# Matrixeigs/PowerSystemsReliabilityAssessment

Hardware: AMD Instinct MI355X
Metric: Monte Carlo DC-OPF scenarios/sec (RTS-24 HL2 non-sequential) (higher is better)
Workload: dtype f64

## Files before the change

powersystemsreliabilityassessment_amd/_lib.py:

```python
from __future__ import annotations

import ctypes as C
import os
import subprocess

from . import _abi

_CSRC = os.path.join(os.path.dirname(os.path.abspath(__file__)), "csrc")
LIB_PATH = os.environ.get("RELMC_LIB_PATH") or os.path.join(_CSRC, "librelmc.so")

EXPORTS = [
    "relmc_ctx_create", "relmc_ctx_destroy", "relmc_last_error", "relmc_version",
    "relmc_solver_opts_default", "relmc_nsq_opts_default", "relmc_case_load",
    "relmc_case_thresholds", "relmc_mc_sampling", "relmc_mc_sampling_dev",
    "relmc_mc_simulation", "relmc_mc_simulation_dev", "relmc_nsq_accumulate", "relmc_nsq_accumulate_distinct",
    "relmc_last_kernel_ms", "relmc_acc_zero", "relmc_acc_merge", "relmc_nsq_indices",
    "relmc_nsq_run", "relmc_hl1_load", "relmc_hl1_nsq", "relmc_hl1_seq_load", "relmc_hl1_seq", "relmc_hl1_seq_events", "relmc_hl1_seq_sweep",
    "relmc_hl1_plan_load", "relmc_hl1_plan", "relmc_hl1_area_load", "relmc_hl1_area", "relmc_hl1_area_tie_outages",
    "relmc_comm_unique_id", "relmc_comm_init", "relmc_comm_allreduce_acc", "relmc_comm_destroy", "relmc_comm_set_host_allreduce", "relmc_comm_info",
    "relmc_db_reset", "relmc_nsq_db_batch", "relmc_db_accumulate", "relmc_db_size", "relmc_db_export", "relmc_db_import",
    "relmc_seq_load", "relmc_seq_mcsampling", "relmc_seq_mcsimulation", "relmc_seq_years", "relmc_retry_stats", "relmc_retry_overflow", "relmc_retry_dense_stats", "relmc_case_order",
    "relmc_case_order_hint", "relmc_tune_order",
    "relmc_comm_set_timeout", "relmc_comm_allreduce_f64", "relmc_comm_set_host_allreduce_f64", "relmc_device_pci_bus_id", "relmc_seq_opts_default", "relmc_seq_run",
    "relmc_is_ratios", "relmc_is_sampling", "relmc_is_sampling_dev", "relmc_nsq_is_accumulate", "relmc_is_acc_zero", "relmc_is_acc_merge", "relmc_nsq_is_indices",
# ... 165 lines not shown
    L.relmc_is_acc_zero.argtypes = [C.POINTER(_abi.IsAcc)]
    L.relmc_is_acc_zero.restype = None
    L.relmc_is_acc_merge.argtypes = [C.POINTER(_abi.IsAcc), C.POINTER(_abi.IsAcc)]
    L.relmc_is_acc_merge.restype = None
    L.relmc_nsq_is_indices.argtypes = [C.POINTER(_abi.IsAcc), C.c_int32, C.c_int32, C.c_double, C.POINTER(_abi.IsIndices)]
    L.relmc_nsq_is_indices.restype = None
    L.relmc_is_tune_opts_default.argtypes = [C.POINTER(_abi.IsTuneOpts)]
    L.relmc_is_tune_opts_default.restype = None
    L.relmc_nsq_is_tune.argtypes = [vp, C.POINTER(_abi.IsTuneOpts), dp, C.POINTER(_abi.IsTuneReport)]
    L.relmc_nsq_is_tune.restype = C.c_int32
    L.relmc_is_run_opts_default.argtypes = [C.POINTER(_abi.IsRunOpts)]
    L.relmc_is_run_opts_default.restype = None
    L.relmc_nsq_is_run.argtypes = [vp, C.POINTER(_abi.IsRunOpts), C.POINTER(_abi.IsRunResult)]
    L.relmc_nsq_is_run.restype = C.c_int32
    if hasattr(L, "relmc_debug_mc_simulation_dense"):
        L.relmc_debug_mc_simulation_dense.argtypes = [vp, u8p, C.c_int64, C.c_void_p, dp, dp, i32p, i32p]
        L.relmc_debug_mc_simulation_dense.restype = C.c_int32
    L.relmc_case_order.argtypes = [vp, i32p, i32p]
    L.relmc_case_order.restype = C.c_int32
    L.relmc_case_order_hint.argtypes = [vp, i32p, C.c_int32]
    L.relmc_case_order_hint.restype = C.c_int32
    L.relmc_tune_order.argtypes = [C.c_void_p, C.c_int32, C.c_uint64, i32p, i32p, i32p]
    L.relmc_tune_order.restype = C.c_int32
    L.relmc_db_export.argtypes = [vp, C.c_int64, C.c_int64, u8p, _abi.c_int64_p, dp, i32p, dp, i32p, i32p, u8p]
    L.relmc_db_export.restype = C.c_int32
    L.relmc_db_import.argtypes = [vp, C.c_void_p, C.c_int64, u8p, _abi.c_int64_p, dp, dp, i32p, i32p, u8p]
    L.relmc_db_import.restype = C.c_int32
    if hasattr(L, "relmc_debug_screen_states"):
        L.relmc_debug_screen_states.argtypes = [vp, u8p, dp, C.c_int64, u8p]
        L.relmc_debug_screen_states.restype = C.c_int32
    if hasattr(L, "relmc_debug_stretch_len"):
        L.relmc_debug_stretch_len.argtypes = [C.c_int64, C.c_int64, C.c_double, C.c_double, C.c_int64, i32p]
        L.relmc_debug_stretch_len.restype = C.c_int64
    if hasattr(L, "relmc_debug_set"):
        L.relmc_debug_set.argtypes = [vp, C.c_char_p, C.c_int32]
        L.relmc_debug_set.restype = C.c_int32
    if hasattr(L, "relmc_debug_tail_plan"):
        L.relmc_debug_tail_plan.argtypes = [C.c_int64, C.c_int32, C.c_void_p, C.c_void_p, C.c_void_p, C.c_void_p]
        L.relmc_debug_tail_plan.restype = C.c_int32
        L.relmc_debug_tail_groups.argtypes = [vp, _abi.c_int64_p, i32p]
        L.relmc_debug_tail_groups.restype = C.c_int32
    if hasattr(L, "relmc_dpp_probe"):
        L.relmc_dpp_probe.argtypes = [vp, dp, dp]
        L.relmc_dpp_probe.restype = C.c_int32
    _lib = L
    return L
```

powersystemsreliabilityassessment_amd/csrc/relmc_ctx.h:

```cpp
#pragma once
#include <hip/hip_runtime.h>

#include <cmath>
#include <cstdint>
#include <functional>
#include <string>
#include <vector>

#include "../../include/relmc.h"
#include "relmc_dev.h"

struct relmc_switches {
    bool no_retry = false;
    bool retry_dense_first = false;
    bool nsq_no_stretch = false;
    bool db_no_probe = false;
    bool dynamic_shape = false;
    bool static_tail = false;
};

namespace relmc_host {
template <class T, bool Pinned = false>
class Buffer {
public:
// ... 151 lines not shown
        c->retry_units = units; c->retry_converged = converged; c->retry_dense_units = dense_units; c->retry_dense_converged = dense_converged; c->retry_overflow = overflow;
    }
};

namespace relmc_host {

using namespace relmc;

extern const char* const kNoCtx;
int fail(relmc_ctx* ctx, int code, const std::string& msg);
bool verbose();
inline int64_t first_non_finite(const double* x, int64_t n)
{
    for (int64_t i = 0; i < n; ++i)
        if (!std::isfinite(x[i])) return i;
    return -1;
}

#define HIP_TRY(ctx, expr)                                                                                   \
    do {                                                                                                     \
        hipError_t e_ = (expr);                                                                              \
        if (e_ != hipSuccess)                                                                                \
            return ::relmc_host::fail(ctx, RELMC_ERR_HIP, std::string(#expr) + ": " + hipGetErrorString(e_)); \
    } while (0)

struct SymOpts {
    const int32_t* order_hint = nullptr; int n_hint = 0;
    int place_moves = 100;
    long place_ww = 1;
    bool no_quarter = false, no_half = false, no_bwd_half = false, no_bus_map = false;
    int scen_pad4 = 0;
    int model_leaf_free = -1;
};
struct SymGeom { uint32_t stash_off = 0, scen_doubles = 0, lds_bytes = 0; long conflict_before = 0, conflict_after = 0; };
SymOpts sym_opts_default();
template <class TL>
int case_symbolic(const relmc_case_desc* d, DevCaseT<TL>& C, int order_variant, const SymOpts& so, SymGeom& geom, std::string& err);
extern template int case_symbolic<Tile24>(const relmc_case_desc*, DevCaseT<Tile24>&, int, const SymOpts&, SymGeom&, std::string&);
extern template int case_symbolic<Tile96>(const relmc_case_desc*, DevCaseT<Tile96>&, int, const SymOpts&, SymGeom&, std::string&);
inline bool fits_tile24(const relmc_case_desc* d)
{
    return d->nb <= Tile24::NBT && d->nl <= Tile24::NLT && d->ng + d->nd <= Tile24::NIT && d->ng + d->nl <= Tile24::NCOMPMAX;
}

EvalArgs make_args(const relmc_solver_opts& o);
int launch_eval(relmc_ctx* ctx, int mode, EvalArgs& a, int* rows_out, hipEvent_t ev_start = nullptr, hipEvent_t ev_stop = nullptr, int alt = 0);
int launch_finalize(relmc_ctx* ctx, int rows);
int finish_timing(relmc_ctx* ctx);
int case_load_image(relmc_ctx* ctx, const relmc_case_desc* d, int order_variant);
inline int mask_words(const relmc_ctx* ctx) { return ctx->tile == 0 ? Tile24::OW : Tile96::OW; }

#ifndef RELMC_TAIL_GROUPS
#define RELMC_TAIL_GROUPS 8
#endif
constexpr int kTailGroups = RELMC_TAIL_GROUPS;
struct TailPlan {
    int64_t ngroups, waves; int T;
    TailPlan(int64_t n, int64_t waves_) : ngroups((n + Tile24::SPW - 1) / Tile24::SPW), waves(waves_), T(waves_ > 0 && ngroups / waves_ >= 2 * kTailGroups ? kTailGroups : 0) {}
    int64_t begin(int64_t w) const { return ngroups * w / waves; }
    int64_t end(int64_t w) const { return ngroups * (w + 1) / waves; }
    int64_t cut(int64_t w) const { return end(w) - T; }
    int64_t items() const { return waves * T; }
    int64_t owner(int64_t p) const { return p % waves; }
    int64_t group(int64_t p) const { return end(p % waves) - T + p / waves; }
};

constexpr uint32_t kFailCapMin = 4096, kFailCapSteady = 1u << 20, kFailCapMax = 1u << 26;
// ... 58 lines not shown
```

powersystemsreliabilityassessment_amd/csrc/relmc_dev.h:

```cpp
#pragma once
#include <stdint.h>

namespace relmc {

template <int RW_, int BS_, int LS_, int IS_, int NCOMPMAX_, int MAXPASS_, int MAXOFF_, int WPB_>
struct TileT {
    static constexpr int RW = RW_;
    static constexpr int BS = BS_;
    static constexpr int LS = LS_;
    static constexpr int IS = IS_;
    static constexpr int NBT = BS_ * RW_;
    static constexpr int NLT = LS_ * RW_;
    static constexpr int NIT = IS_ * RW_;
    static constexpr int SPW = 64 / RW_;
    static constexpr int NCOMPMAX = NCOMPMAX_;
    static constexpr int OW = NCOMPMAX_ / 32;
    static constexpr int MAXPASS = MAXPASS_;
    static constexpr int MAXOFF = MAXOFF_;
    static constexpr int WPB = WPB_;
    static_assert(BS_ <= 2 && LS_ <= 3 && IS_ <= 4, "the per-lane flag word has room for 2 bus, 3 line and 4 injection slots");
};
using Tile24 = TileT<16, 2, 3, 4, 128, 96, 160, 4>;
using Tile96 = TileT<64, 2, 2, 3, 256, 64, 320, 8>;
constexpr int DEGMAX = 8;
constexpr int BINJMAX = 8;

constexpr uint32_t LF_EXISTS = 1u, LF_OWNER = 2u, LF_LIMITED = 4u;
constexpr uint32_t IK_NONE = 0u, IK_REAL = 1u, IK_VIRTUAL = 2u;

template <class TL>
struct DevCaseT {
    static constexpr int NBT = TL::NBT, NLT = TL::NLT, NIT = TL::NIT, NCOMPMAX = TL::NCOMPMAX, MAXPASS = TL::MAXPASS, MAXOFF = TL::MAXOFF, ROWL = TL::RW;
    int32_t nb, ng, nl, nd, ninj, ncomp, ref_bus, noff;
    double base_mva, total_load;
    uint32_t exist_mask;
    uint32_t nws;
    uint16_t off_rhs, off_p;
    uint16_t npass, npass_upd, npass_inv, nzero;
    uint16_t maxdeg, maxinj, base_connected, npass_updq;
    uint16_t maxdeg_s[2], maxinj_s[2];
    uint16_t npass_updh, pad3[3];
    uint64_t bwd_half;
    uint64_t b_line8[NBT];
    uint64_t b_inj8[NBT];
    double b_bsum[NBT];
    double l_b[NLT];
    double l_rate[NLT];
    uint32_t l_info[NLT];
    int32_t l_partner[NLT];
    uint16_t l_blk[NLT];
    alignas(16) double i_tab[NIT][4];
    uint32_t i_info[NIT];
    uint8_t b_nline[NBT];
    uint8_t b_line[NBT][DEGMAX];
    uint8_t b_ninj[NBT];
    uint8_t b_inj[NBT][BINJMAX];
    int16_t b_vinj[NBT];
    uint8_t b_ext[NBT];
    uint8_t b_lane[NBT];
    uint8_t b_int[NBT];
    uint32_t thr[NCOMPMAX];
// ... 153 lines not shown
```

powersystemsreliabilityassessment_amd/csrc/relmc_kernels.hip:

```cpp
#include "relmc_devfn.h"
#include "relmc_shape_rts24.h"

namespace relmc {


constexpr int kPrioBit = 12;
constexpr int kMinWaves = 2;
#define DINF __builtin_inf()
#define RELOAD_FENCE() __asm__ volatile("" ::: "memory")
#define SLOT_FENCE() __builtin_amdgcn_sched_barrier(0)
#ifdef RELMC_PASS_NOUNROLL
#define PASS_LOOP _Pragma("nounroll")
#else
#define PASS_LOOP
#endif
constexpr int kPfMask = 0xc0;
constexpr int kPfMaskWide = 0xc6;
#define PFSITE(k) (((PF_MASK >> (k)) & 1) != 0)
#ifdef RELMC_PHASE_TIMING
#define PT_DECL unsigned long long pt_[8] = {0, 0, 0, 0, 0, 0, 0, 0}; unsigned long long pt0_ = __builtin_readcyclecounter();
#define PT_MARK(k) { const unsigned long long n_ = __builtin_readcyclecounter(); pt_[k] += n_ - pt0_; pt0_ = n_; }
#define PT_FLUSH if (a.timing && lane == 0) { for (int k = 0; k < 8; ++k) a.timing[((size_t)blockIdx.x * WPB + (tid >> 6)) * 8 + k] = pt_[k]; }
#else
#define PT_DECL
#define PT_MARK(k)
#define PT_FLUSH
#endif
#if defined(RELMC_PHASE_TIMING) && defined(RELMC_PT_INIT)
#undef PT_MARK
#define PT_MARK(k) { const unsigned long long n_ = __builtin_readcyclecounter(); pt_[(k) == 7 ? 7 : 6] += n_ - pt0_; pt0_ = n_; }
#define PT_IMARK(k) { const unsigned long long n_ = __builtin_readcyclecounter(); pt_[k] += n_ - pt0_; pt0_ = n_; }
#else
#define PT_IMARK(k)
#endif

template <int MODE_, class TL, class SH = ShapeDynamic>
__global__ void __launch_bounds__(64 * TL::WPB, kMinWaves) relmc_eval_kernel(const DevCaseT<TL>* __restrict__ gcase, const EvalArgs a)
{
    constexpr int MODE = MODE_ == 5 ? 0 : (MODE_ == 6 ? 4 : MODE_);
    constexpr bool DENSE = MODE_ == 6;
    constexpr int PAIR_MASK = TL::RW == 16 ? kRpairMask : kRpairMaskWide;
#define PAIRSITE(k) (((PAIR_MASK >> (k)) & 1) != 0)
    constexpr int PF_MASK = TL::RW == 16 ? kPfMask : kPfMaskWide;
    constexpr int RW = TL::RW, BS = TL::BS, LS = TL::LS, IS = TL::IS, NBT = TL::NBT, WPB = TL::WPB, SPW = TL::SPW, OW = TL::OW;
    using DevCase = DevCaseT<TL>;
    using Partial = PartialT<TL>;
    extern __shared__ __attribute__((aligned(16))) unsigned char smem[];
    constexpr uint32_t OPT_BYTES = 128;
    double* const OPT = reinterpret_cast<double*>(smem);
#define A_(k, name) OPT[k]
    DevCase& C = *reinterpret_cast<DevCase*>(smem + OPT_BYTES);
    const DevCase& TASKSRC = *gcase;
    const DevCase& TABL = C;
    const DevCase& TABI = (RW == 64) ? *gcase : C;
    const DevCase& TABG = (RW == 64) ? *gcase : C;
    const int tid = threadIdx.x, lane = tid & 63, rlane = lane & (RW - 1), row = tid / RW;
    const uint32_t case_bytes = a.case_bytes;
    {
        const uint32_t* src = reinterpret_cast<const uint32_t*>(gcase);
        uint32_t* dst = reinterpret_cast<uint32_t*>(smem + OPT_BYTES);
        if (tid == 0) { OPT[0] = a.feastol; OPT[1] = a.gradtol; OPT[2] = a.comptol; OPT[3] = a.costtol; OPT[4] = a.xi; OPT[5] = a.sigma;
                        OPT[6] = a.z0; OPT[7] = a.alpha_min; OPT[8] = a.max_stepsize; OPT[9] = a.fail_threshold; }
        for (uint32_t i = tid; i < case_bytes / 4; i += 64 * WPB) dst[i] = src[i];
    }
    __syncthreads();
    double* const W = reinterpret_cast<double*>(smem + OPT_BYTES + ((case_bytes + 15u) & ~15u)) + (size_t)row * SHAPE(scen_doubles, a.scen_doubles);
    const int nlp = SHAPE(nl, C.nl), nip = SHAPE(ninj, C.ninj);
    double* const LR = W;
    double* const IR = W + 4 * (nlp + 1);
    const int maxdeg0 = SHAPE(maxdeg0, C.maxdeg_s[0]), maxdeg1 = SHAPE(maxdeg1, C.maxdeg_s[1]), maxinj0 = SHAPE(maxinj0, C.maxinj_s[0]), maxinj1 = SHAPE(maxinj1, C.maxinj_s[1]);
    double* const Stash = W + SHAPE(stash_off, a.stash_off) + 2 * rlane;
    const double* const StashJ = W + SHAPE(stash_off, a.stash_off);
    double* const Lam = W + SHAPE(stash_off, a.stash_off) + 2 * IS * RW + 2;
    uint32_t* const OB = reinterpret_cast<uint32_t*>(Lam + NBT);

    const int ng = SHAPE(ng, C.ng), ncomp = C.ncomp, nb = SHAPE(nb, C.nb);
// ... 741 lines not shown
                        for (int i = k + rlane; i < n; i += RW) { const double v = __builtin_fabs(A[(size_t)i * n1 + k]); if (v > best) { best = v; bi = i; } }
                        const double mx = row_max<RW>(best);
                        const uint32_t cand = (best == mx) ? (uint32_t)bi : (uint32_t)n;
                        const int p = (int)row_min_u32<RW>(cand);
                        if (!(mx > 0.0)) { singular_k = true; break; }
                        if (p != k) for (int j = k + rlane; j <= n; j += RW) { const double u = A[(size_t)k * n1 + j], v = A[(size_t)p * n1 + j]; A[(size_t)k * n1 + j] = v; A[(size_t)p * n1 + j] = u; }
                        __threadfence_block();
                        const double rp = 1.0 / A[(size_t)k * n1 + k];
                        for (int i = k + 1 + rlane; i < n; i += RW) Fm[i] = A[(size_t)i * n1 + k] * rp;
                        RELOAD_FENCE();
                        for (int i = k + 1; i < n; ++i) {
                            const double f = Fm[i];
                            if (f != 0.0) for (int j = k + 1 + rlane; j <= n; j += RW) A[(size_t)i * n1 + j] = A[(size_t)i * n1 + j] - f * A[(size_t)k * n1 + j];
                        }
                        __threadfence_block();
                    }
                    for (int k = n - 1; k >= 0 && !singular_k; --k) {
                        double sdot = 0.0;
                        for (int j = k + 1 + rlane; j < n; j += RW) sdot = __builtin_fma(A[(size_t)k * n1 + j], Fm[j], sdot);
                        sdot = row_sum<RW>(sdot);
                        if (rlane == 0) Fm[k] = (A[(size_t)k * n1 + n] - sdot) / A[(size_t)k * n1 + k];
                        RELOAD_FENCE();
                    }
                    double xs[(2 * NBT + RW - 1) / RW];
#pragma unroll
                    for (int q = 0; q < (2 * NBT + RW - 1) / RW; ++q) { const int e = rlane + RW * q; xs[q] = e < n ? (singular_k ? __builtin_nan("") : Fm[e]) : 0.0; }
                    RELOAD_FENCE();
#pragma unroll
                    for (int q = 0; q < (2 * NBT + RW - 1) / RW; ++q) { const int e = rlane + RW * q; if (e < n) W[off_rhs + e] = xs[q]; }
                    RELOAD_FENCE();
                } else {
                unsigned char* const W8 = reinterpret_cast<unsigned char*>(W);
#define WP(off) reinterpret_cast<double*>(W8 + (off))
                uint2 dsc = *reinterpret_cast<const uint2*>(&TASKSRC.task[0][rlane][0]);
                PASS_LOOP
                for (int p = 0; p < npuf; ++p) {
                    const uint2 nxt = *reinterpret_cast<const uint2*>(&TASKSRC.task[p + 1][rlane][0]);
                    if ((dsc.x & 0xffffu) != 0xffffu) {
                        const bool vec = (dsc.x & 0x8000u) != 0;
                        double* T = WP(dsc.x & 0x7fffu);
                        const double* Wa = WP(dsc.x >> 16);
                        const double* Wb = WP(dsc.y & 0xffffu);
                        const double* D = WP(dsc.y >> 16);
                        const d2 dA = ld2(D); const double dBy = D[3];
                        const d2 a0 = ld2(Wa), b0 = ld2(Wb), b1 = ld2(Wb + 2);
                        d2 t0 = ld2(T);
                        const double pm = dA.x, pb = dA.y, pe = -dBy;
                        const double q = frcp(__builtin_fma(pm, pe, pb * pb));
                        const double P00 = pe * q, P01 = pb * q, P11 = -pm * q;
                        const double g00 = __builtin_fma(a0.x, P00, a0.y * P01), g01 = __builtin_fma(a0.x, P01, a0.y * P11);
                        t0.x -= __builtin_fma(g00, b0.x, g01 * b0.y); t0.y -= __builtin_fma(g00, b1.x, g01 * b1.y);
                        st2(T, t0.x, t0.y);
                        if (!vec) {
                            const d2 a1 = ld2(Wa + 2);
                            d2 t1 = ld2(T + 2);
                            const double g10 = __builtin_fma(a1.x, P00, a1.y * P01), g11 = __builtin_fma(a1.x, P01, a1.y * P11);
                            t1.x -= __builtin_fma(g10, b0.x, g11 * b0.y); t1.y -= __builtin_fma(g10, b1.x, g11 * b1.y);
                            st2(T + 2, t1.x, t1.y);
                        }
                    }
                    dsc = nxt;
                }
                PASS_LOOP
                for (int p = npuf; p < npuh; ++p) {
                    const uint2 nxt = *reinterpret_cast<const uint2*>(&TASKSRC.task[p + 1][rlane][0]);
                    if ((dsc.x & 0xffffu) != 0xffffu) {
                        double* T = WP(dsc.x & 0xffffu);
                        const double* Wa = WP(dsc.x >> 16);
                        const double* Wb = WP(dsc.y & 0xffffu);
                        const double* D = WP(dsc.y >> 16);
                        const d2 dA = ld2(D); const double dBy = D[3];
                        const d2 a0 = ld2(Wa), b0 = ld2(Wb), b1 = ld2(Wb + 2);
                        d2 t0 = ld2(T);
                        const double pm = dA.x, pb = dA.y, pe = -dBy;
                        const double q = frcp(__builtin_fma(pm, pe, pb * pb));
                        const double P00 = pe * q, P01 = pb * q, P11 = -pm * q;
                        const double g00 = __builtin_fma(a0.x, P00, a0.y * P01), g01 = __builtin_fma(a0.x, P01, a0.y * P11);
                        t0.x -= __builtin_fma(g00, b0.x, g01 * b0.y); t0.y -= __builtin_fma(g00, b1.x, g01 * b1.y);
                        st2(T, t0.x, t0.y);
                    }
                    dsc = nxt;
                }
                PASS_LOOP
                for (int p = npuh; p < npu; ++p) {
                    const uint2 nxt = *reinterpret_cast<const uint2*>(&TASKSRC.task[p + 1][rlane][0]);
                    if ((dsc.x & 0xffffu) != 0xffffu) {
                        double* T = WP(dsc.x & 0xffffu);
                        const double* Wa = WP(dsc.x >> 16);
                        const double* Wb = WP(dsc.y & 0xffffu);
                        const double* D = WP(dsc.y >> 16);
                        const d2 dA = ld2(D); const double dBy = D[3];
                        const d2 a0 = ld2(Wa), b0 = ld2(Wb);
                        double t = *T;
                        const double pm = dA.x, pb = dA.y, pe = -dBy;
                        const double q = frcp(__builtin_fma(pm, pe, pb * pb));
                        const double P00 = pe * q, P01 = pb * q, P11 = -pm * q;
                        const double g0 = __builtin_fma(a0.x, P00, a0.y * P01), g1 = __builtin_fma(a0.x, P01, a0.y * P11);
                        t -= __builtin_fma(g0, b0.x, g1 * b0.y);
                        *T = t;
                    }
                    dsc = nxt;
                }
                PT_MARK(4)
                PASS_LOOP
                for (int p = npu; p < npu + npi; ++p) {
                    const uint2 nxt = *reinterpret_cast<const uint2*>(&TASKSRC.task[p + 1][rlane][0]);
                    if ((dsc.x & 0xffffu) != 0xffffu) {
                        double* D = WP(dsc.x & 0xffffu);
                        double* Y = WP(dsc.x >> 16);
                        const d2 dA = ld2(D), y = ld2(Y); const double dBy = D[3];
                        const double pm = dA.x, pb = dA.y, pe = -dBy;
                        const double q = frcp(__builtin_fma(pm, pe, pb * pb));
                        const double P00 = pe * q, P01 = pb * q, P11 = -pm * q;
                        st2(D, P00, P01); st2(D + 2, P01, P11);
                        st2(Y, __builtin_fma(P00, y.x, P01 * y.y), __builtin_fma(P01, y.x, P11 * y.y));
                    }
                    dsc = nxt;
                }
                PT_MARK(5)
                if (RW == 64 && bwd_all_half) {
                PASS_LOOP
                    for (int p = npu + npi; p < npass; ++p) {
                        const uint2 nxt = *reinterpret_cast<const uint2*>(&TASKSRC.task[p + 1][rlane][0]);
                        if ((dsc.x & 0xffffu) != 0xffffu) {
                            double* Yi = WP(dsc.x & 0xffffu);
                            const double* Wk = WP(dsc.x >> 16);
                            const double* Pr = WP(dsc.y & 0xffffu);
                            const double* Ya = WP(dsc.y >> 16);
                            const d2 w0 = ld2(Wk), w1 = ld2(Wk + 2), pr = ld2(Pr), x = ld2(Ya);
                            double y = *Yi;
                            const double u0 = __builtin_fma(w0.x, x.x, w1.x * x.y), u1 = __builtin_fma(w0.y, x.x, w1.y * x.y);
                            y -= __builtin_fma(pr.x, u0, pr.y * u1);
                            *Yi = y;
                        }
                        dsc = nxt;
                    }
                } else
                PASS_LOOP
                for (int p = npu + npi; p < npass; ++p) {
                    const uint2 nxt = *reinterpret_cast<const uint2*>(&TASKSRC.task[p + 1][rlane][0]);
                    if ((dsc.x & 0xffffu) != 0xffffu) {
                        double* Yi = WP(dsc.x & 0xffffu);
                        const double* Wk = WP(dsc.x >> 16);
                        const double* P = WP(dsc.y & 0xffffu);
                        const double* Ya = WP(dsc.y >> 16);
                        const d2 w0 = ld2(Wk), w1 = ld2(Wk + 2), p0 = ld2(P), p1 = ld2(P + 2), x = ld2(Ya);
                        d2 y = ld2(Yi);
                        const double u0 = __builtin_fma(w0.x, x.x, w1.x * x.y), u1 = __builtin_fma(w0.y, x.x, w1.y * x.y);
                        y.x -= __builtin_fma(p0.x, u0, p0.y * u1); y.y -= __builtin_fma(p1.x, u0, p1.y * u1);
                        st2(Yi, y.x, y.y);
                    }
                    dsc = nxt;
                }
                PT_MARK(5)
                }
                RELOAD_FENCE();
                const double* X = W + off_rhs;
                double step2 = 0.0;
                double dth[BS], dla[BS];
#pragma unroll
                for (int t = 0; t < BS; ++t) {
                    const int bi = vb[t];
                    dth[t] = 0; dla[t] = 0;
                    if (bi < nb) { const d2 x = ld2(X + 2 * bi); dth[t] = x.x; dla[t] = x.y; step2 = __builtin_fma(x.x, x.x, __builtin_fma(x.y, x.y, step2)); }
                }
                double tp = 0.0, td = 0.0;
                double dF[LS], dG[LS];
                double dpv[IS];
                double o_ms = 0.0;
                if constexpr (PFSITE(6)) o_ms = A_(8, max_stepsize);
                if constexpr (PFSITE(3)) {
                    d2 xf[LS], xt[LS], sh[IS]; double dlb[IS];
#pragma unroll
                    for (int s = 0; s < LS; ++s) { xf[s] = ld2(X + 2 * (linfo[s] & 0xff)); xt[s] = ld2(X + 2 * ((linfo[s] >> 8) & 0xff)); }
#pragma unroll
                    for (int s = 0; s < IS; ++s) { dlb[s] = X[2 * (iinfo[s] & 0xff) + 1]; sh[s] = ld2(Stash + 2 * RW * s); }
#pragma unroll
                    for (int s = 0; s < LS; ++s) { dF[s] = L_ON(s) ? lb(s) * (xf[s].x - xt[s].x) : 0.0; dG[s] = L_ON(s) ? lb(s) * (xf[s].y - xt[s].y) : 0.0; }
#pragma unroll
                    for (int s = 0; s < IS; ++s) dpv[s] = I_BOX(s) ? __builtin_fma(dlb[s], sh[s].x, -sh[s].y) : 0.0;
                }
#pragma unroll
                for (int s = 0; s < LS; ++s) {
// ... 335 lines not shown
```

powersystemsreliabilityassessment_amd/csrc/relmc_schedule.hip:

```cpp
#include <algorithm>
#include <chrono>
#include <cmath>
#include <cstddef>
#include <cstdio>
#include <cstdlib>
#include <cstring>
#include <memory>

#include "relmc_ctx.h"
#ifdef RELMC_DEV_SWITCHES
#include "relmc_dev_switches.h"
#endif

namespace relmc_host {

bool verbose()
{
    static const bool v = std::getenv("RELMC_VERBOSE") != nullptr;
    return v;
}

SymOpts sym_opts_default()
{
    SymOpts so;
// ... 225 lines not shown
                std::vector<int> remaining;
                for (int i = 0; i < nt; ++i) if (tasks[i].kind == kind) remaining.push_back(i);
                while (!remaining.empty()) {
                    const int cur = (int)pkind.size();
                    if (cur >= MAXPASS - 1) return failx(RELMC_ERR_UNSUPPORTED, "relmc_case_load: solver schedule exceeds MAXPASS");
                    std::vector<int> ready;
                    for (int i : remaining) {
                        bool ok = true;
                        for (int q : strict[i]) if (passof[q] < 0 || passof[q] >= cur) { ok = false; break; }
                        if (ok) ready.push_back(i);
                    }
                    std::stable_sort(ready.begin(), ready.end(), [&](int a2, int b2) { return depth[a2] != depth[b2] ? depth[a2] > depth[b2] : a2 < b2; });
                    std::vector<int> chosen;
                    std::vector<char> in_pass(nt, 0);
                    const int cap = (kind == 0 && cur >= best_f) ? ROWL / 2 : ROWL;
                    for (int i : ready) {
                        if ((int)chosen.size() >= cap) break;
                        bool ok = true;
                        for (int q : weak[i]) if (passof[q] < 0 && !in_pass[q]) { ok = false; break; }
                        if (ok) { chosen.push_back(i); in_pass[i] = 1; }
                    }
                    if (chosen.empty()) return failx(RELMC_ERR_INVALID, "relmc_case_load: solver schedule has a dependency cycle");
                    pkind.push_back(kind); pcount.push_back((int)chosen.size()); pass_tasks.push_back(std::vector<int>(ROWL, -1));
                    for (size_t k = 0; k < chosen.size(); ++k) { pass_tasks[cur][k] = chosen[k]; passof[chosen[k]] = cur; }
                    std::vector<int> rest;
                    for (int i : remaining) if (passof[i] < 0) rest.push_back(i);
                    remaining.swap(rest);
                }
            }
        }
        (void)lastw; (void)lastr;
        const auto t_place0 = std::chrono::steady_clock::now();
        if (verbose()) fprintf(stderr, "relmc: scheduling %.1f ms\n", std::chrono::duration<double, std::milli>(t_place0 - t_sched0).count());
        {
            const uint32_t eval_d = 4u * (nl + 1) + 4u * (ninj + 1);
            uint32_t stride = C.nws > eval_d ? C.nws : eval_d;
            stride = (stride + 1u) & ~1u;
            stride += 2u * IS * ROWL + 2u + NBT + OW / 2u;
            while ((stride & 3u) != 2u) stride += 1;
            stride += 4u * (uint32_t)so.scen_pad4;
            static const int kGroupOfLane[64] = {0,0,0,0,1,1,1,1,1,1,1,1,0,0,0,0, 1,1,1,1,0,0,0,0,0,0,0,0,1,1,1,1,
                                                 2,2,2,2,3,3,3,3,3,3,3,3,2,2,2,2, 3,3,3,3,2,2,2,2,2,2,2,2,3,3,3,3};
            auto remap = [&](int o) {
                const int f = o & 0x8000; o &= 0x7fff;
                if (o >= 4 * nb && o < (int)C.off_rhs) o = 4 * pos[o >> 2] + (o & 3);
                return o | f;
            };
            const long ww = so.place_ww;
            auto pass_cost = [&](int p) {
                long cost = 0;
                const int kind = pkind[p];
                const int nins = kind == 0 ? 8 : (kind == 1 ? 3 : 6);
                for (int ins = 0; ins < nins; ++ins) {
                    int cnt[4][16]; int addr[4][16][16];
                    for (int g = 0; g < 4; ++g) for (int q = 0; q < 16; ++q) cnt[g][q] = 0;
                    for (int lane = 0; lane < 64; ++lane) {
                        const int slot = lane % ROWL, row = lane / ROWL;
                        const int ti = pass_tasks[p][slot];
                        if (ti < 0) continue;
                        const Task& t = tasks[ti];
                        int o = -1;
                        if (kind == 0) {
                            const bool vec = (t.o[0] & 0x8000) != 0;
                            switch (ins) {
                                case 0: o = remap(t.o[3]); break;            case 1: o = remap(t.o[3]) + 2; break;
                                case 2: o = remap(t.o[1]); break;            case 3: o = remap(t.o[2]); break;
                                case 4: o = remap(t.o[2]) + 2; break;        case 5: o = remap(t.o[0]) & 0x7fff; break;
                                case 6: if (!vec) o = remap(t.o[1]) + 2; break;
                                default: if (!vec) o = (remap(t.o[0]) & 0x7fff) + 2; break;
                            }
                        } else if (kind == 1) {
                            o = ins == 0 ? remap(t.o[0]) : (ins == 1 ? remap(t.o[0]) + 2 : remap(t.o[1]));
                        } else {
                            switch (ins) {
                                case 0: o = remap(t.o[1]); break; case 1: o = remap(t.o[1]) + 2; break;
// ... 101 lines not shown
            }
        }
        C.bwd_half = 0;
        if (!so.no_bwd_half) {
            int first_bwd = 0;
            while (first_bwd < (int)pkind.size() && pkind[first_bwd] != 2) first_bwd++;
            bool all_half = ROWL == 64 && (int)pkind.size() - first_bwd <= 64 && first_bwd < (int)pkind.size();
            for (int p = first_bwd; p < (int)pkind.size(); ++p) if (pcount[p] > ROWL / 2) all_half = false;
            for (int p = first_bwd; all_half && p < (int)pkind.size(); ++p) {
                uint16_t full[ROWL][4]; int nfull = 0;
                for (int r = 0; r < ROWL; ++r) if (C.task[p][r][0] != 0xffff) { for (int k = 0; k < 4; ++k) full[nfull][k] = C.task[p][r][k]; nfull++; }
                for (int r = 0; r < ROWL; ++r) for (int k = 0; k < 4; ++k) C.task[p][r][k] = 0xffff;
                for (int t = 0; t < nfull; ++t)
                    for (int r = 0; r < 2; ++r) {
                        uint16_t* q = C.task[p][2 * t + r];
                        q[0] = (uint16_t)(full[t][0] + r); q[1] = full[t][1]; q[2] = (uint16_t)(full[t][2] + 2 * r); q[3] = full[t][3];
                    }
                C.bwd_half |= 1ull << (p - first_bwd);
            }
        }
        {
            int nup_all = 0;
            for (size_t q = 0; q < pkind.size(); ++q) if (pkind[q] == 0) nup_all++;
            const int nfull_upd = nup_all - (int)C.npass_updq - (int)C.npass_updh;
            for (size_t q = 0; q < pkind.size(); ++q)
                for (int r = 0; r < ROWL; ++r) {
                    if (C.task[q][r][0] == 0xffff) continue;
                    for (int k = 0; k < 4; ++k) {
                        const uint32_t v = C.task[q][r][k], f = (k == 0 && (int)q < nfull_upd) ? (v & 0x8000u) : 0u;
                        C.task[q][r][k] = (uint16_t)(((v & (f ? 0x7fffu : 0xffffu)) << 3) | f);
                    }
                }
        }
        C.npass = (uint16_t)pkind.size();
        int nu = 0, ni = 0;
        for (size_t q = 0; q < pkind.size(); ++q) {
            C.pass_ntask[q] = (uint8_t)pcount[q];
            if (pkind[q] == 0) nu++; else if (pkind[q] == 1) ni++;
            if (q > 0 && pkind[q] < pkind[q - 1]) return failx(RELMC_ERR_INVALID, "relmc_case_load: schedule phases out of order");
        }
        C.npass_upd = (uint16_t)nu; C.npass_inv = (uint16_t)ni;
        if (verbose()) { fprintf(stderr, "relmc: order %d: %d + %d + %d passes, tasks per pass:", order_variant, nu, ni, (int)pkind.size() - nu - ni); for (size_t q = 0; q < pkind.size(); ++q) fprintf(stderr, " %d", pcount[q]); fprintf(stderr, "\n"); }
    }

    for (int l = 0; l < NLT; ++l) C.l_partner[l] = -1;
    std::vector<int> pair_owner((size_t)nb * nb, -1), pair_lines((size_t)nb * nb, 0);
    std::vector<char> has_line(nb + noff, 0);
    for (int l = 0; l < nl; ++l) {
        const int f = ext2int[d->br_from[l]], t = ext2int[d->br_to[l]];
        const int lo = f < t ? f : t, hi = f < t ? t : f;
        uint32_t flags = LF_EXISTS;
        if (d->br_rate[l] != 0.0) flags |= LF_LIMITED;
        const size_t key = (size_t)hi * nb + lo;
        if (pair_owner[key] < 0) {
            pair_owner[key] = l; flags |= LF_OWNER;
            if (blk[hi][lo] < 0) return failx(RELMC_ERR_INVALID, "relmc_case_load: line outside the symbolic pattern");
            C.l_blk[l] = (uint16_t)OFFB(hi, lo);
            has_line[blk[hi][lo]] = 1;
        } else {
            if (pair_lines[key] >= 2) return failx(RELMC_ERR_UNSUPPORTED, "relmc_case_load: more than two parallel lines");
            C.l_partner[pair_owner[key]] = l;
        }
        pair_lines[key]++;
        C.l_b[l] = d->br_b[l];
        C.l_rate[l] = d->br_rate[l] / d->base_mva;
        C.l_info[l] = (uint32_t)f | ((uint32_t)t << 8) | (flags << 24);
// ... 159 lines not shown

using namespace relmc_host;

extern "C" {

int32_t relmc_tune_order(const relmc_case_desc* d, int32_t evaluations, uint64_t seed, const int32_t* start, int32_t* order_out, int32_t stats_out[4])
{
    if (!d || !order_out || evaluations < 0 || d->nb < 1) return RELMC_ERR_INVALID;
    if (fits_tile24(d)) return tune_order_impl<Tile24>(d, evaluations, seed, start, order_out, stats_out);
    return tune_order_impl<Tile96>(d, evaluations, seed, start, order_out, stats_out);
}

int32_t relmc_debug_symbolic(const relmc_case_desc* d, int32_t order_variant, const int32_t* order_hint, int32_t n_hint, int32_t* hdr, uint16_t* tasks, int64_t tasks_cap, uint8_t* pass_ntask,
                             uint8_t* b_int, uint16_t* l_blk, uint32_t* l_info, uint16_t* zero_off, char* err, int32_t err_cap, int32_t model_leaf_free)
{
    if (!d || !hdr || !tasks || !pass_ntask || !b_int || !l_blk || !l_info || !zero_off) return RELMC_ERR_INVALID;
    SymOpts so = sym_opts_default();
    if (order_hint && n_hint > 0) { so.order_hint = order_hint; so.n_hint = n_hint; }
    if (model_leaf_free >= 0) so.model_leaf_free = model_leaf_free;
    std::string errs;
    SymGeom g;
    int rc;
    auto dump = [&](const auto& C, int tile, int rw, int maxpass) {
        for (int k = 0; k < 24; ++k) hdr[k] = 0;
        hdr[0] = tile; hdr[1] = rw; hdr[2] = C.nb; hdr[3] = C.noff; hdr[4] = (int)C.nws; hdr[5] = C.off_rhs; hdr[6] = C.npass; hdr[7] = C.npass_upd;
        hdr[8] = C.npass_inv; hdr[9] = C.npass_updh; hdr[10] = C.npass_updq; hdr[11] = C.nzero; hdr[12] = (int)g.scen_doubles; hdr[13] = (int)g.lds_bytes;
        hdr[14] = (int)g.conflict_before; hdr[15] = (int)g.conflict_after; hdr[16] = maxpass; hdr[17] = C.nl;
        hdr[19] = (int32_t)(uint32_t)(C.bwd_half & 0xffffffffull); hdr[20] = (int32_t)(uint32_t)(C.bwd_half >> 32);
        hdr[21] = (int32_t)((uint32_t)C.maxdeg_s[0] | ((uint32_t)C.maxdeg_s[1] << 8) | ((uint32_t)C.maxinj_s[0] << 16) | ((uint32_t)C.maxinj_s[1] << 24));
        if ((int64_t)C.npass * rw * 4 > tasks_cap) return (int)RELMC_ERR_INVALID;
        for (int p = 0; p < C.npass; ++p) { pass_ntask[p] = C.pass_ntask[p]; for (int r = 0; r < rw; ++r) for (int k = 0; k < 4; ++k) {
            const uint16_t v = C.task[p][r][k];
            const bool full_upd = p < C.npass_upd - C.npass_updh - C.npass_updq;
            tasks[((size_t)p * rw + r) * 4 + k] = C.task[p][r][0] == 0xffff ? v : (uint16_t)((k == 0 && full_upd) ? (((v & 0x7fffu) >> 3) | (v & 0x8000u)) : (v >> 3));
        } }
        for (int i = 0; i < C.nb; ++i) b_int[i] = C.b_int[i];
        for (int l = 0; l < C.nl; ++l) { l_info[l] = C.l_info[l]; l_blk[l] = ((C.l_info[l] >> 24) & LF_OWNER) ? C.l_blk[l] : (uint16_t)0xffff; }
        for (int z = 0; z < C.nzero; ++z) zero_off[z] = C.zero_off[z];
        return (int)RELMC_OK;
    };
    if (fits_tile24(d)) {
        auto C = std::make_unique<DevCaseT<Tile24>>();
        rc = case_symbolic<Tile24>(d, *C, order_variant, so, g, errs);
        if (rc == RELMC_OK) rc = dump(*C, 0, Tile24::RW, Tile24::MAXPASS);
    } else {
        auto C = std::make_unique<DevCaseT<Tile96>>();
        rc = case_symbolic<Tile96>(d, *C, order_variant, so, g, errs);
        if (rc == RELMC_OK) rc = dump(*C, 1, Tile96::RW, Tile96::MAXPASS);
    }
    if (err && err_cap > 0) { std::strncpy(err, errs.c_str(), (size_t)err_cap - 1); err[err_cap - 1] = 0; }
    return rc;
}

}
```

Before: 61.15 million.

## Let idle solver lanes shadow active tasks to align LDS accesses

```diff
diff --git a/powersystemsreliabilityassessment_amd/_lib.py b/powersystemsreliabilityassessment_amd/_lib.py
--- a/powersystemsreliabilityassessment_amd/_lib.py
+++ b/powersystemsreliabilityassessment_amd/_lib.py
@@ -221,6 +221,9 @@
     if hasattr(L, "relmc_debug_stretch_len"):
         L.relmc_debug_stretch_len.argtypes = [C.c_int64, C.c_int64, C.c_double, C.c_double, C.c_int64, i32p]
         L.relmc_debug_stretch_len.restype = C.c_int64
+    if hasattr(L, "relmc_debug_task_image"):
+        L.relmc_debug_task_image.argtypes = [C.c_void_p, C.c_int32, C.c_void_p, C.c_int32, C.c_void_p, C.c_void_p, C.c_int64, C.c_char_p, C.c_int32]
+        L.relmc_debug_task_image.restype = C.c_int32
     if hasattr(L, "relmc_debug_set"):
         L.relmc_debug_set.argtypes = [vp, C.c_char_p, C.c_int32]
         L.relmc_debug_set.restype = C.c_int32
diff --git a/powersystemsreliabilityassessment_amd/csrc/relmc_ctx.h b/powersystemsreliabilityassessment_amd/csrc/relmc_ctx.h
--- a/powersystemsreliabilityassessment_amd/csrc/relmc_ctx.h
+++ b/powersystemsreliabilityassessment_amd/csrc/relmc_ctx.h
@@ -207,7 +207,8 @@
     int scen_pad4 = 0;
     int model_leaf_free = -1;
 };
-struct SymGeom { uint32_t stash_off = 0, scen_doubles = 0, lds_bytes = 0; long conflict_before = 0, conflict_after = 0; };
+struct SymGeom { uint32_t stash_off = 0, scen_doubles = 0, lds_bytes = 0; long conflict_before = 0, conflict_after = 0;
+                 long shadow_masked = 0, shadow_tasks = 0, shadow_all = 0; };
 SymOpts sym_opts_default();
 template <class TL>
 int case_symbolic(const relmc_case_desc* d, DevCaseT<TL>& C, int order_variant, const SymOpts& so, SymGeom& geom, std::string& err);
diff --git a/powersystemsreliabilityassessment_amd/csrc/relmc_dev.h b/powersystemsreliabilityassessment_amd/csrc/relmc_dev.h
--- a/powersystemsreliabilityassessment_amd/csrc/relmc_dev.h
+++ b/powersystemsreliabilityassessment_amd/csrc/relmc_dev.h
@@ -27,6 +27,9 @@
 
 constexpr uint32_t LF_EXISTS = 1u, LF_OWNER = 2u, LF_LIMITED = 4u;
 constexpr uint32_t IK_NONE = 0u, IK_REAL = 1u, IK_VIRTUAL = 2u;
+
+constexpr uint16_t TASK_IDLE_INV = 0xffff;
+inline bool task_idle(const uint16_t* t, bool inv) { return inv ? (t[2] | t[3]) != 0 : t[0] == t[3]; }
 
 template <class TL>
 struct DevCaseT {
diff --git a/powersystemsreliabilityassessment_amd/csrc/relmc_kernels.hip b/powersystemsreliabilityassessment_amd/csrc/relmc_kernels.hip
--- a/powersystemsreliabilityassessment_amd/csrc/relmc_kernels.hip
+++ b/powersystemsreliabilityassessment_amd/csrc/relmc_kernels.hip
@@ -17,6 +17,10 @@
 constexpr int kPfMask = 0xc0;
 constexpr int kPfMaskWide = 0xc6;
 #define PFSITE(k) (((PF_MASK >> (k)) & 1) != 0)
+constexpr int kShadowMask = 0xff;
+constexpr int kShadowMaskWide = 0xff;
+#define PASS_IDLE(d) (((d).x & 0xffffu) == ((d).y >> 16))
+#define PASS_IDLE_INV(d) ((d).y != 0u)
 #ifdef RELMC_PHASE_TIMING
 #define PT_DECL unsigned long long pt_[8] = {0, 0, 0, 0, 0, 0, 0, 0}; unsigned long long pt0_ = __builtin_readcyclecounter();
 #define PT_MARK(k) { const unsigned long long n_ = __builtin_readcyclecounter(); pt_[k] += n_ - pt0_; pt0_ = n_; }
@@ -42,6 +46,7 @@
     constexpr int PAIR_MASK = TL::RW == 16 ? kRpairMask : kRpairMaskWide;
 #define PAIRSITE(k) (((PAIR_MASK >> (k)) & 1) != 0)
     constexpr int PF_MASK = TL::RW == 16 ? kPfMask : kPfMaskWide;
+    constexpr bool SHADOW = (((TL::RW == 16 ? kShadowMask : kShadowMaskWide) >> MODE) & 1) != 0;
     constexpr int RW = TL::RW, BS = TL::BS, LS = TL::LS, IS = TL::IS, NBT = TL::NBT, WPB = TL::WPB, SPW = TL::SPW, OW = TL::OW;
     using DevCase = DevCaseT<TL>;
     using Partial = PartialT<TL>;
@@ -849,11 +854,13 @@
                 } else {
                 unsigned char* const W8 = reinterpret_cast<unsigned char*>(W);
 #define WP(off) reinterpret_cast<double*>(W8 + (off))
+#define SHADOW_PIN(...) do { if constexpr (SHADOW) __asm__ volatile("" :: __VA_ARGS__ : "memory"); } while (0)
                 uint2 dsc = *reinterpret_cast<const uint2*>(&TASKSRC.task[0][rlane][0]);
                 PASS_LOOP
                 for (int p = 0; p < npuf; ++p) {
                     const uint2 nxt = *reinterpret_cast<const uint2*>(&TASKSRC.task[p + 1][rlane][0]);
-                    if ((dsc.x & 0xffffu) != 0xffffu) {
+                    const bool idle = PASS_IDLE(dsc);
+                    if (SHADOW || !idle) {
                         const bool vec = (dsc.x & 0x8000u) != 0;
                         double* T = WP(dsc.x & 0x7fffu);
                         const double* Wa = WP(dsc.x >> 16);
@@ -867,13 +874,13 @@
                         const double P00 = pe * q, P01 = pb * q, P11 = -pm * q;
                         const double g00 = __builtin_fma(a0.x, P00, a0.y * P01), g01 = __builtin_fma(a0.x, P01, a0.y * P11);
                         t0.x -= __builtin_fma(g00, b0.x, g01 * b0.y); t0.y -= __builtin_fma(g00, b1.x, g01 * b1.y);
-                        st2(T, t0.x, t0.y);
-                        if (!vec) {
+                        SHADOW_PIN("v"(t0.x), "v"(t0.y)); if (!idle) st2(T, t0.x, t0.y);
+                        if (SHADOW || !vec) {
                             const d2 a1 = ld2(Wa + 2);
                             d2 t1 = ld2(T + 2);
                             const double g10 = __builtin_fma(a1.x, P00, a1.y * P01), g11 = __builtin_fma(a1.x, P01, a1.y * P11);
                             t1.x -= __builtin_fma(g10, b0.x, g11 * b0.y); t1.y -= __builtin_fma(g10, b1.x, g11 * b1.y);
-                            st2(T + 2, t1.x, t1.y);
+                            SHADOW_PIN("v"(t1.x), "v"(t1.y)); if (!idle && !vec) st2(T + 2, t1.x, t1.y);
                         }
                     }
                     dsc = nxt;
@@ -881,7 +888,8 @@
                 PASS_LOOP
                 for (int p = npuf; p < npuh; ++p) {
                     const uint2 nxt = *reinterpret_cast<const uint2*>(&TASKSRC.task[p + 1][rlane][0]);
-                    if ((dsc.x & 0xffffu) != 0xffffu) {
+                    const bool idle = PASS_IDLE(dsc);
+                    if (SHADOW || !idle) {
                         double* T = WP(dsc.x & 0xffffu);
                         const double* Wa = WP(dsc.x >> 16);
                         const double* Wb = WP(dsc.y & 0xffffu);
@@ -894,14 +902,15 @@
                         const double P00 = pe * q, P01 = pb * q, P11 = -pm * q;
                         const double g00 = __builtin_fma(a0.x, P00, a0.y * P01), g01 = __builtin_fma(a0.x, P01, a0.y * P11);
                         t0.x -= __builtin_fma(g00, b0.x, g01 * b0.y); t0.y -= __builtin_fma(g00, b1.x, g01 * b1.y);
-                        st2(T, t0.x, t0.y);
+                        SHADOW_PIN("v"(t0.x), "v"(t0.y)); if (!idle) st2(T, t0.x, t0.y);
                     }
                     dsc = nxt;
                 }
                 PASS_LOOP
                 for (int p = npuh; p < npu; ++p) {
                     const uint2 nxt = *reinterpret_cast<const uint2*>(&TASKSRC.task[p + 1][rlane][0]);
-                    if ((dsc.x & 0xffffu) != 0xffffu) {
+                    const bool idle = PASS_IDLE(dsc);
+                    if (SHADOW || !idle) {
                         double* T = WP(dsc.x & 0xffffu);
                         const double* Wa = WP(dsc.x >> 16);
                         const double* Wb = WP(dsc.y & 0xffffu);
@@ -914,7 +923,7 @@
                         const double P00 = pe * q, P01 = pb * q, P11 = -pm * q;
                         const double g0 = __builtin_fma(a0.x, P00, a0.y * P01), g1 = __builtin_fma(a0.x, P01, a0.y * P11);
                         t -= __builtin_fma(g0, b0.x, g1 * b0.y);
-                        *T = t;
+                        SHADOW_PIN("v"(t)); if (!idle) *T = t;
                     }
                     dsc = nxt;
                 }
@@ -922,15 +931,16 @@
                 PASS_LOOP
                 for (int p = npu; p < npu + npi; ++p) {
                     const uint2 nxt = *reinterpret_cast<const uint2*>(&TASKSRC.task[p + 1][rlane][0]);
-                    if ((dsc.x & 0xffffu) != 0xffffu) {
+                    const bool idle = PASS_IDLE_INV(dsc);
+                    if (SHADOW || !idle) {
                         double* D = WP(dsc.x & 0xffffu);
                         double* Y = WP(dsc.x >> 16);
                         const d2 dA = ld2(D), y = ld2(Y); const double dBy = D[3];
                         const double pm = dA.x, pb = dA.y, pe = -dBy;
                         const double q = frcp(__builtin_fma(pm, pe, pb * pb));
                         const double P00 = pe * q, P01 = pb * q, P11 = -pm * q;
-                        st2(D, P00, P01); st2(D + 2, P01, P11);
-                        st2(Y, __builtin_fma(P00, y.x, P01 * y.y), __builtin_fma(P01, y.x, P11 * y.y));
+                        const double y0 = __builtin_fma(P00, y.x, P01 * y.y), y1 = __builtin_fma(P01, y.x, P11 * y.y);
+                        SHADOW_PIN("v"(P00), "v"(P01), "v"(P11), "v"(y0), "v"(y1)); if (!idle) { st2(D, P00, P01); st2(D + 2, P01, P11); st2(Y, y0, y1); }
                     }
                     dsc = nxt;
                 }
@@ -939,7 +949,8 @@
                 PASS_LOOP
                     for (int p = npu + npi; p < npass; ++p) {
                         const uint2 nxt = *reinterpret_cast<const uint2*>(&TASKSRC.task[p + 1][rlane][0]);
-                        if ((dsc.x & 0xffffu) != 0xffffu) {
+                        const bool idle = PASS_IDLE(dsc);
+                        if (SHADOW || !idle) {
                             double* Yi = WP(dsc.x & 0xffffu);
                             const double* Wk = WP(dsc.x >> 16);
                             const double* Pr = WP(dsc.y & 0xffffu);
@@ -948,7 +959,7 @@
                             double y = *Yi;
                             const double u0 = __builtin_fma(w0.x, x.x, w1.x * x.y), u1 = __builtin_fma(w0.y, x.x, w1.y * x.y);
                             y -= __builtin_fma(pr.x, u0, pr.y * u1);
-                            *Yi = y;
+                            SHADOW_PIN("v"(y)); if (!idle) *Yi = y;
                         }
                         dsc = nxt;
                     }
@@ -956,7 +967,8 @@
                 PASS_LOOP
                 for (int p = npu + npi; p < npass; ++p) {
                     const uint2 nxt = *reinterpret_cast<const uint2*>(&TASKSRC.task[p + 1][rlane][0]);
-                    if ((dsc.x & 0xffffu) != 0xffffu) {
+                    const bool idle = PASS_IDLE(dsc);
+                    if (SHADOW || !idle) {
                         double* Yi = WP(dsc.x & 0xffffu);
                         const double* Wk = WP(dsc.x >> 16);
                         const double* P = WP(dsc.y & 0xffffu);
@@ -965,7 +977,7 @@
                         d2 y = ld2(Yi);
                         const double u0 = __builtin_fma(w0.x, x.x, w1.x * x.y), u1 = __builtin_fma(w0.y, x.x, w1.y * x.y);
                         y.x -= __builtin_fma(p0.x, u0, p0.y * u1); y.y -= __builtin_fma(p1.x, u0, p1.y * u1);
-                        st2(Yi, y.x, y.y);
+                        SHADOW_PIN("v"(y.x), "v"(y.y)); if (!idle) st2(Yi, y.x, y.y);
                     }
                     dsc = nxt;
                 }
diff --git a/powersystemsreliabilityassessment_amd/csrc/relmc_schedule.hip b/powersystemsreliabilityassessment_amd/csrc/relmc_schedule.hip
--- a/powersystemsreliabilityassessment_amd/csrc/relmc_schedule.hip
+++ b/powersystemsreliabilityassessment_amd/csrc/relmc_schedule.hip
@@ -281,15 +281,16 @@
         (void)lastw; (void)lastr;
         const auto t_place0 = std::chrono::steady_clock::now();
         if (verbose()) fprintf(stderr, "relmc: scheduling %.1f ms\n", std::chrono::duration<double, std::milli>(t_place0 - t_sched0).count());
+        static const int kGroupOfLane[64] = {0,0,0,0,1,1,1,1,1,1,1,1,0,0,0,0, 1,1,1,1,0,0,0,0,0,0,0,0,1,1,1,1,
+                                             2,2,2,2,3,3,3,3,3,3,3,3,2,2,2,2, 3,3,3,3,2,2,2,2,2,2,2,2,3,3,3,3};
+        uint32_t stride = 0;
         {
             const uint32_t eval_d = 4u * (nl + 1) + 4u * (ninj + 1);
-            uint32_t stride = C.nws > eval_d ? C.nws : eval_d;
+            stride = C.nws > eval_d ? C.nws : eval_d;
             stride = (stride + 1u) & ~1u;
             stride += 2u * IS * ROWL + 2u + NBT + OW / 2u;
             while ((stride & 3u) != 2u) stride += 1;
             stride += 4u * (uint32_t)so.scen_pad4;
-            static const int kGroupOfLane[64] = {0,0,0,0,1,1,1,1,1,1,1,1,0,0,0,0, 1,1,1,1,0,0,0,0,0,0,0,0,1,1,1,1,
-                                                 2,2,2,2,3,3,3,3,3,3,3,3,2,2,2,2, 3,3,3,3,2,2,2,2,2,2,2,2,3,3,3,3};
             auto remap = [&](int o) {
                 const int f = o & 0x8000; o &= 0x7fff;
                 if (o >= 4 * nb && o < (int)C.off_rhs) o = 4 * pos[o >> 2] + (o & 3);
@@ -457,6 +458,84 @@
                     }
                 }
         }
+        {
+            const int np = (int)pkind.size();
+            int nup_all = 0;
+            for (int q = 0; q < np; ++q) if (pkind[q] == 0) nup_all++;
+            const int nfull_upd = nup_all - (int)C.npass_updq - (int)C.npass_updh, nhalf_end = nup_all - (int)C.npass_updq;
+            int first_bwd = 0;
+            while (first_bwd < np && pkind[first_bwd] != 2) first_bwd++;
+            static const int kRdFull[8][2] = {{3, 0}, {3, 16}, {1, 0}, {2, 0}, {2, 16}, {0, 0}, {1, 16}, {0, 16}};
+            static const int kRdHalf[6][2] = {{3, 0}, {3, 16}, {1, 0}, {2, 0}, {2, 16}, {0, 0}};
+            static const int kRdQuarter[5][2] = {{3, 0}, {3, 16}, {1, 0}, {2, 0}, {0, 0}};
+            static const int kRdInv[3][2] = {{0, 0}, {0, 16}, {1, 0}};
+            static const int kRdBwd[6][2] = {{1, 0}, {1, 16}, {2, 0}, {2, 16}, {3, 0}, {0, 0}};
+            static const int kRdBwdHalf[5][2] = {{1, 0}, {1, 16}, {2, 0}, {3, 0}, {0, 0}};
+            auto form_of = [&](int p, const int (*&rd)[2]) {
+                if (pkind[p] == 0) { if (p < nfull_upd) { rd = kRdFull; return 8; } if (p < nhalf_end) { rd = kRdHalf; return 6; } rd = kRdQuarter; return 5; }
+                if (pkind[p] == 1) { rd = kRdInv; return 3; }
+                if ((C.bwd_half >> (p - first_bwd)) & 1) { rd = kRdBwdHalf; return 5; }
+                rd = kRdBwd; return 6;
+            };
+            auto image_cost = [&](int p, int mode) {
+                const bool all = mode == 2;
+                const int (*rd)[2] = nullptr; const int nins = form_of(p, rd);
+                const bool inv = pkind[p] == 1, full = pkind[p] == 0 && p < nfull_upd;
+                long cost = 0;
+                for (int ins = 0; ins < nins; ++ins) {
+                    int cnt[4][16]; int addr[4][16][16];
+                    for (int g = 0; g < 4; ++g) for (int q = 0; q < 16; ++q) cnt[g][q] = 0;
+                    for (int lane = 0; lane < 64; ++lane) {
+                        const uint16_t* t = C.task[p][lane % ROWL];
+                        if (t[0] == 0xffff && t[3] == 0xffff) continue;
+                        if (!all && (task_idle(t, inv) || (mode == 0 && full && ins >= 6 && (t[0] & 0x8000u)))) continue;
+                        const int f = rd[ins][0], o = (int)((f == 0 && full) ? (t[0] & 0x7fffu) : t[f]) + rd[ins][1];
+                        const int ad = (lane / ROWL) * (int)stride * 8 + o, g = kGroupOfLane[lane], q = (ad >> 4) & 15;
+                        bool seen = false;
+                        for (int k = 0; k < cnt[g][q]; ++k) if (addr[g][q][k] == ad) { seen = true; break; }
+                        if (!seen) addr[g][q][cnt[g][q]++] = ad;
+                    }
+                    for (int g = 0; g < 4; ++g) { int mx = 0; for (int q = 0; q < 16; ++q) if (cnt[g][q] > mx) mx = cnt[g][q]; if (mx > 1) cost += mx - 1; }
+                }
+                return cost;
+            };
+            long masked = 0, tasks_all_rows = 0, shadowed = 0;
+            const bool model = so.place_moves > 0;
+            for (int p = 0; p < np; ++p) {
+                const bool inv = pkind[p] == 1;
+                std::vector<int> active;
+                for (int r = 0; r < ROWL; ++r) {
+                    const uint16_t* t = C.task[p][r];
+                    if (t[0] == 0xffff) continue;
+                    if (task_idle(t, inv)) return failx(RELMC_ERR_INVALID, "relmc_case_load: a solver task carries the idle marker");
+                    active.push_back(r);
+                }
+                if (active.empty()) return failx(RELMC_ERR_INVALID, "relmc_case_load: a solver pass without a task");
+                if (model) { masked += image_cost(p, 0); tasks_all_rows += image_cost(p, 1); }
+                const int ngroup = ROWL == 64 ? 4 : 2;
+                for (int g = 0; g < ngroup; ++g) {
+                    std::vector<int> idle;
+                    for (int r = 0; r < ROWL; ++r) if (C.task[p][r][0] == 0xffff && kGroupOfLane[r] == g) idle.push_back(r);
+                    if (idle.empty()) continue;
+                    std::vector<int> cand;
+                    for (int r : active) if (kGroupOfLane[r] == g) cand.push_back(r);
+                    if (cand.empty()) cand = active;
+                    auto assign = [&](int src) {
+                        for (int r : idle) {
+                            uint16_t* q = C.task[p][r]; const uint16_t* s = C.task[p][src];
+                            if (inv) { q[0] = s[0]; q[1] = s[1]; q[2] = TASK_IDLE_INV; q[3] = TASK_IDLE_INV; }
+                            else { q[0] = s[3]; q[1] = s[1]; q[2] = s[2]; q[3] = s[3]; }
+                        }
+                    };
+                    int best = -1; long bestc = 0;
+                    for (int src : cand) { if (!model) { best = src; break; } assign(src); const long c = image_cost(p, 2); if (best < 0 || c < bestc) { best = src; bestc = c; } }
+                    assign(best);
+                }
+                if (model) shadowed += image_cost(p, 2);
+            }
+            geom.shadow_masked = masked; geom.shadow_tasks = tasks_all_rows; geom.shadow_all = shadowed;
+            if (verbose()) fprintf(stderr, "relmc: order %d: modelled LDS conflict cycles of the device image, idle lanes masked %ld, the tasks with every second row read %ld, idle lanes shadowing %ld\n", order_variant, masked, tasks_all_rows, shadowed);
+        }
         C.npass = (uint16_t)pkind.size();
         int nu = 0, ni = 0;
         for (size_t q = 0; q < pkind.size(); ++q) {
@@ -682,7 +761,8 @@
         for (int p = 0; p < C.npass; ++p) { pass_ntask[p] = C.pass_ntask[p]; for (int r = 0; r < rw; ++r) for (int k = 0; k < 4; ++k) {
             const uint16_t v = C.task[p][r][k];
             const bool full_upd = p < C.npass_upd - C.npass_updh - C.npass_updq;
-            tasks[((size_t)p * rw + r) * 4 + k] = C.task[p][r][0] == 0xffff ? v : (uint16_t)((k == 0 && full_upd) ? (((v & 0x7fffu) >> 3) | (v & 0x8000u)) : (v >> 3));
+            const bool inv = p >= C.npass_upd && p < C.npass_upd + C.npass_inv;
+            tasks[((size_t)p * rw + r) * 4 + k] = task_idle(C.task[p][r], inv) ? (uint16_t)0xffff : (uint16_t)((k == 0 && full_upd) ? (((v & 0x7fffu) >> 3) | (v & 0x8000u)) : (v >> 3));
         } }
         for (int i = 0; i < C.nb; ++i) b_int[i] = C.b_int[i];
         for (int l = 0; l < C.nl; ++l) { l_info[l] = C.l_info[l]; l_blk[l] = ((C.l_info[l] >> 24) & LF_OWNER) ? C.l_blk[l] : (uint16_t)0xffff; }
@@ -702,4 +782,35 @@
     return rc;
 }
 
-}
+int32_t relmc_debug_task_image(const relmc_case_desc* d, int32_t order_variant, const int32_t* order_hint, int32_t n_hint, int32_t* hdr, uint16_t* tasks, int64_t tasks_cap,
+                               char* err, int32_t err_cap)
+{
+    if (!d || !hdr || !tasks) return RELMC_ERR_INVALID;
+    SymOpts so = sym_opts_default();
+    if (order_hint && n_hint > 0) { so.order_hint = order_hint; so.n_hint = n_hint; }
+    std::string errs;
+    SymGeom g;
+    int rc;
+    auto dump = [&](const auto& C, int tile, int rw) {
+        for (int k = 0; k < 16; ++k) hdr[k] = 0;
+        hdr[0] = tile; hdr[1] = rw; hdr[2] = C.nb; hdr[3] = (int)C.nws; hdr[4] = C.off_rhs; hdr[5] = C.npass; hdr[6] = C.npass_upd; hdr[7] = C.npass_inv;
+        hdr[8] = C.npass_updh; hdr[9] = C.npass_updq; hdr[10] = (int32_t)(uint32_t)(C.bwd_half & 0xffffffffull); hdr[11] = (int32_t)(uint32_t)(C.bwd_half >> 32);
+        hdr[12] = (int)g.scen_doubles; hdr[13] = (int)g.shadow_masked; hdr[14] = (int)g.shadow_all; hdr[15] = (int)g.shadow_tasks;
+        if ((int64_t)C.npass * rw * 4 > tasks_cap) return (int)RELMC_ERR_INVALID;
+        for (int p = 0; p < C.npass; ++p) for (int r = 0; r < rw; ++r) for (int k = 0; k < 4; ++k) tasks[((size_t)p * rw + r) * 4 + k] = C.task[p][r][k];
+        return (int)RELMC_OK;
+    };
+    if (fits_tile24(d)) {
+        auto C = std::make_unique<DevCaseT<Tile24>>();
+        rc = case_symbolic<Tile24>(d, *C, order_variant, so, g, errs);
+        if (rc == RELMC_OK) rc = dump(*C, 0, Tile24::RW);
+    } else {
+        auto C = std::make_unique<DevCaseT<Tile96>>();
+        rc = case_symbolic<Tile96>(d, *C, order_variant, so, g, errs);
+        if (rc == RELMC_OK) rc = dump(*C, 1, Tile96::RW);
+    }
+    if (err && err_cap > 0) { std::strncpy(err, errs.c_str(), (size_t)err_cap - 1); err[err_cap - 1] = 0; }
+    return rc;
+}
+
+}
```

New measurement: 61.86 million, median of 6. 1.01x the previous value.
